# samiwilf/torchrec-oldfork

Hardware: AMD Instinct MI355X
Metric: samples/sec Criteo-1TB DLRM batch 65536 (higher is better)
Workload: dtype f32; 1 GPU; DLRM Criteo-1TB shape: 26 tables (177.9M rows, 84.85 GiB fp32, D=128), 13 dense, pooling factor 1, dense 512-256-128, over 1024-1024-512-256-1, fused exact SGD; global_batch=65536, local_batch=65536, parallelism=mp1: 26 table-wise + 0 row-wise + 0 replicated (data-parallel) tables, dense dp1, ids=uniform, distinct_batches=32, seed=0, data_ranks=1

## Files before the change

### torchrec-oldfork_amd/csrc/dlrm_interaction.hip

```cpp
#include <algorithm>
#include <cstdlib>

#include "common.hpp"

namespace tbe {

using f32x4 = __attribute__((ext_vector_type(4))) float;

__device__ __forceinline__ void wave_lds_fence() { __builtin_amdgcn_wave_barrier(); }

__device__ __forceinline__ int triu_index(int i, int j, int R) { return i * (2 * R - i - 1) / 2 + (j - i - 1); }

__device__ __forceinline__ int triu_row(int p, int R) {
  const int t = 2 * R - 1;
  int i = static_cast<int>((static_cast<float>(t) - sqrtf(static_cast<float>(t * t - 8 * p))) * 0.5f);
  i = max(0, min(i, R - 2));
  while (i + 1 <= R - 2 && (i + 1) * (2 * R - (i + 1) - 1) / 2 <= p) ++i;
  while (i > 0 && i * (2 * R - i - 1) / 2 > p) --i;
  return i;
}

template <int D>
struct XLoader {
  static constexpr int LOG_V = (D == 16 ? 2 : D == 32 ? 3 : D == 64 ? 4 : D == 128 ? 5 : 6);
  __device__ static __forceinline__ const float* src(const float* dense, const float* sparse, int64_t b, int F, int v) {
    const int r = v >> LOG_V;
    const int c = (v & ((1 << LOG_V) - 1)) * 4;
    return r == 0 ? dense + b * D + c : sparse + (b * F + (r - 1)) * D + c;
  }
};

template <int D>
__global__ __launch_bounds__(256, (D <= 128 ? 4 : 2)) void interaction_fwd_kernel(const float* __restrict__ dense,
                                                                                  const float* __restrict__ sparse,
                                                                                  float* __restrict__ out, int B, int F,
                                                                                  int64_t out_stride) {
  extern __shared__ float smem[];
  constexpr int NS = D / 16;
  const int lane = threadIdx.x & 63;
  const int wave = threadIdx.x >> 6;
  const int R = F + 1;
  const int P = R * (R - 1) / 2;
  const int P4 = (P + 3) & ~3;
  float* zs = smem + wave * P4;
  const bool vec_out = (out_stride & 3) == 0 && out_stride >= D + P4 && (reinterpret_cast<uintptr_t>(out) & 15) == 0;
  if (lane < P4 - P) zs[P + lane] = 0.f;
  const int r16 = lane & 15;
  const int kq = lane >> 4;
  const int row0 = min(r16, R - 1);
  const int row1 = min(16 + r16, R - 1);
  const int stride_b = gridDim.x * 4;
  float4 xa[NS], xb[NS];
  float4 dpass = make_float4(0.f, 0.f, 0.f, 0.f);
  auto issue_loads = [&](int b) {
    const float* x0 = (row0 == 0 ? dense + static_cast<int64_t>(b) * D
                                 : sparse + (static_cast<int64_t>(b) * F + (row0 - 1)) * D) + 4 * kq;
    const float* x1 = sparse + (static_cast<int64_t>(b) * F + (row1 - 1)) * D + 4 * kq;
#pragma unroll
    for (int s = 0; s < NS; ++s) xa[s] = ld4(x0 + 16 * s);
    if (R > 16) {
#pragma unroll
      for (int s = 0; s < NS; ++s) xb[s] = ld4(x1 + 16 * s);
    } else {
#pragma unroll
      for (int s = 0; s < NS; ++s) xb[s] = make_float4(0.f, 0.f, 0.f, 0.f);
    }
    if (lane < D / 4) dpass = ld4(dense + static_cast<int64_t>(b) * D + lane * 4);
  };
  int b = blockIdx.x * 4 + wave;
  if (b < B) issue_loads(b);
  for (; b < B; b += stride_b) {
    f32x4 acc00 = {0.f, 0.f, 0.f, 0.f}, acc01 = acc00, acc11 = acc00;
#pragma unroll
    for (int s = 0; s < NS; ++s) {
      const float a0[4] = {xa[s].x, xa[s].y, xa[s].z, xa[s].w};
      const float a1[4] = {xb[s].x, xb[s].y, xb[s].z, xb[s].w};
#pragma unroll
      for (int e = 0; e < 4; ++e) {
        acc00 = __builtin_amdgcn_mfma_f32_16x16x4f32(a0[e], a0[e], acc00, 0, 0, 0);
        acc01 = __builtin_amdgcn_mfma_f32_16x16x4f32(a0[e], a1[e], acc01, 0, 0, 0);
        acc11 = __builtin_amdgcn_mfma_f32_16x16x4f32(a1[e], a1[e], acc11, 0, 0, 0);
      }
    }
    float* orow = out + static_cast<int64_t>(b) * out_stride;
    if (lane < D / 4) {
      if (vec_out) {
        st4(orow + lane * 4, dpass);
      } else {
        orow[lane * 4 + 0] = dpass.x;
        orow[lane * 4 + 1] = dpass.y;
        orow[lane * 4 + 2] = dpass.z;
        orow[lane * 4 + 3] = dpass.w;
      }
    }
    if (b + stride_b < B) issue_loads(b + stride_b);
#pragma unroll
    for (int q = 0; q < 4; ++q) {
      const int i = kq * 4 + q;
      const int j = r16;
      if (i < j && j < R) zs[triu_index(i, j, R)] = acc00[q];
      if (16 + j < R && i < R) zs[triu_index(i, 16 + j, R)] = acc01[q];
      if (i < j && 16 + j < R) zs[triu_index(16 + i, 16 + j, R)] = acc11[q];
    }
    __builtin_amdgcn_wave_barrier();
    constexpr int MAXT = 8;
    constexpr int MAXQ = 2;
    if (vec_out) {
#pragma unroll
      for (int t = 0; t < MAXQ; ++t) {
        const int q = lane + t * kWave;
        if (q < P4 / 4) st4(orow + D + 4 * q, *reinterpret_cast<const float4*>(zs + 4 * q));
      }
    } else {
#pragma unroll
      for (int t = 0; t < MAXT; ++t) {
        const int p = lane + t * kWave;
        if (p < P) orow[D + p] = zs[p];
      }
    }
    __builtin_amdgcn_wave_barrier();
  }
}

__device__ __forceinline__ void vm_store_dword(float* p, float v) {
  asm volatile("global_store_dword %0, %1, off" ::"v"(p), "v"(v) : "memory");
}

template <int N>
__device__ __forceinline__ void vm_wait_all_but() {
  asm volatile("s_waitcnt vmcnt(%0)" ::"n"(N) : "memory");
}

__device__ __forceinline__ void vm_wait_all_but(int n) {
  switch (n) {
    case 1: vm_wait_all_but<1>(); break;
    case 2: vm_wait_all_but<2>(); break;
    case 3: vm_wait_all_but<3>(); break;
    case 4: vm_wait_all_but<4>(); break;
    case 5: vm_wait_all_but<5>(); break;
    case 6: vm_wait_all_but<6>(); break;
    case 7: vm_wait_all_but<7>(); break;
    case 8: vm_wait_all_but<8>(); break;
    case 9: vm_wait_all_but<9>(); break;
    case 10: vm_wait_all_but<10>(); break;
    case 11: vm_wait_all_but<11>(); break;
    case 12: vm_wait_all_but<12>(); break;
    default: vm_wait_all_but<0>(); break;
  }
}

template <int D>
__global__ __launch_bounds__(256, 2) void interaction_fwd_glds_kernel(const float* __restrict__ dense,
                                                                     const float* __restrict__ sparse,
                                                                     float* __restrict__ out, int B, int F,
                                                                     int64_t out_stride) {
  extern __shared__ float smem[];
  constexpr int NS = D / 16;
  constexpr int PR = D / 4;
  constexpr int RPI = kWave / PR;
  constexpr int MAXI = 32 / RPI;
  static_assert(PR >= 16 && PR <= kWave, "LDS-DMA form needs 64 <= D <= 256");
  const int lane = threadIdx.x & 63;
  const int wave = threadIdx.x >> 6;
  const int R = F + 1;
  const int P = R * (R - 1) / 2;
  const int P4 = (P + 3) & ~3;
  const int NI = (R + RPI - 1) / RPI;
  float* xs = smem + wave * (NI * RPI * D + P4);
  float* zs = xs + NI * RPI * D;
  const bool vec_out = (out_stride & 3) == 0 && out_stride >= D + P4 && (reinterpret_cast<uintptr_t>(out) & 15) == 0;
  if (lane < P4 - P) zs[P + lane] = 0.f;
  const int r16 = lane & 15;
  const int kq = lane >> 4;
  const int row0 = min(r16, R - 1);
  const int row1 = min(16 + r16, R - 1);
  const int stride_b = gridDim.x * 4;
  int src_off[MAXI];
#pragma unroll
  for (int i = 0; i < MAXI; ++i) {
    const int row = min(i * RPI + lane / PR, R - 1);
    const int piece = (lane % PR) ^ (row & 15);
    src_off[i] = (row - 1) * D + 4 * piece;
  }
  const bool dense_lane = lane < PR;
  auto issue_copy = [&](int b) {
    const float* sp = sparse + static_cast<int64_t>(b) * F * D;
    const float* dn = dense + static_cast<int64_t>(b) * D + D;
#pragma unroll
    for (int i = 0; i < MAXI; ++i) {
      if (i < NI) {
        const float* g = (i == 0 && dense_lane) ? dn + src_off[0] : sp + src_off[i];
        __builtin_amdgcn_global_load_lds((const __attribute__((address_space(1))) void*)g,
                                         (__attribute__((address_space(3))) void*)(xs + i * (kWave * 4)), 16, 0, 0);
      }
    }
  };
  const int T = (P + kWave - 1) / kWave;
  constexpr int DS = (D + kWave - 1) / kWave;
  int stores_behind_copy = 0;
  int b = blockIdx.x * 4 + wave;
  if (b < B) issue_copy(b);
  for (; b < B; b += stride_b) {
    vm_wait_all_but(stores_behind_copy);
    __builtin_amdgcn_wave_barrier();
    float4 xa[NS], xb[NS];
#pragma unroll
    for (int s = 0; s < NS; ++s) xa[s] = *reinterpret_cast<const float4*>(xs + row0 * D + 4 * ((4 * s + kq) ^ (row0 & 15)));
    if (R > 16) {
#pragma unroll
      for (int s = 0; s < NS; ++s) xb[s] = *reinterpret_cast<const float4*>(xs + row1 * D + 4 * ((4 * s + kq) ^ (row1 & 15)));
    } else {
#pragma unroll
      for (int s = 0; s < NS; ++s) xb[s] = make_float4(0.f, 0.f, 0.f, 0.f);
    }
    float4 dpass = make_float4(0.f, 0.f, 0.f, 0.f);
    float dscal[DS];
    if (vec_out) {
      if (dense_lane) dpass = *reinterpret_cast<const float4*>(xs + 4 * lane);
    } else {
#pragma unroll
      for (int t = 0; t < DS; ++t) dscal[t] = xs[min(lane + t * kWave, D - 1)];
    }
    asm volatile("s_waitcnt lgkmcnt(0)" ::: "memory");
    __builtin_amdgcn_wave_barrier();
    if (b + stride_b < B) issue_copy(b + stride_b);
    f32x4 acc00 = {0.f, 0.f, 0.f, 0.f}, acc01 = acc00, acc11 = acc00;
#pragma unroll
    for (int s = 0; s < NS; ++s) {
      const float a0[4] = {xa[s].x, xa[s].y, xa[s].z, xa[s].w};
      const float a1[4] = {xb[s].x, xb[s].y, xb[s].z, xb[s].w};
#pragma unroll
      for (int e = 0; e < 4; ++e) {
        acc00 = __builtin_amdgcn_mfma_f32_16x16x4f32(a0[e], a0[e], acc00, 0, 0, 0);
        acc01 = __builtin_amdgcn_mfma_f32_16x16x4f32(a0[e], a1[e], acc01, 0, 0, 0);
        acc11 = __builtin_amdgcn_mfma_f32_16x16x4f32(a1[e], a1[e], acc11, 0, 0, 0);
      }
    }
    float* orow = out + static_cast<int64_t>(b) * out_stride;
    if (vec_out) {
      if (dense_lane) st4(orow + lane * 4, dpass);
    } else {
#pragma unroll
      for (int t = 0; t < DS; ++t) vm_store_dword(orow + min(lane + t * kWave, D - 1), dscal[t]);
    }
#pragma unroll
    for (int q = 0; q < 4; ++q) {
      const int i = kq * 4 + q;
      const int j = r16;
      if (i < j && j < R) zs[triu_index(i, j, R)] = acc00[q];
      if (16 + j < R && i < R) zs[triu_index(i, 16 + j, R)] = acc01[q];
      if (i < j && 16 + j < R) zs[triu_index(16 + i, 16 + j, R)] = acc11[q];
    }
    __builtin_amdgcn_wave_barrier();
    constexpr int MAXT = 8;
    constexpr int MAXQ = 2;
    if (vec_out) {
#pragma unroll
      for (int t = 0; t < MAXQ; ++t) {
        const int q = lane + t * kWave;
        if (q < P4 / 4) st4(orow + D + 4 * q, *reinterpret_cast<const float4*>(zs + 4 * q));
      }
      stores_behind_copy = 0;
    } else {
      float zv[MAXT];
#pragma unroll
      for (int t = 0; t < MAXT; ++t)
        if (t < T) zv[t] = zs[min(lane + t * kWave, P - 1)];
#pragma unroll
      for (int t = 0; t < MAXT; ++t)
        if (t < T) vm_store_dword(orow + D + min(lane + t * kWave, P - 1), zv[t]);
      stores_behind_copy = DS + T;
    }
    __builtin_amdgcn_wave_barrier();
  }
}

template <int NT>
__global__ __launch_bounds__(256, 2) void interaction_bwd_kernel(const float* __restrict__ dense,
                                                                 const float* __restrict__ sparse,
                                                                 const float* __restrict__ grad_out,
                                                                 float* __restrict__ grad_dense,
                                                                 float* __restrict__ grad_sparse, int B, int F,
                                                                 int64_t grad_stride) {
  extern __shared__ float smem[];
  constexpr int D = NT * 16;
  constexpr int XS = D + 16;
  constexpr int GS = 34;
  constexpr int XROWS = 28;
  constexpr int LOG_V = XLoader<D>::LOG_V;
  constexpr int MAXV = (XROWS * D / 4 + kWave - 1) / kWave;
  const int lane = threadIdx.x & 63;
  const int wave = threadIdx.x >> 6;
  const int R = F + 1;
  const int P = R * (R - 1) / 2;
  float* xs = smem + wave * (XROWS * XS + 32 * GS);
  float* gs = xs + XROWS * XS;
  const int r16 = lane & 15;
  const int kq = lane >> 4;
  const int nvec = R * (D / 4);
  const int ksteps = (R + 3) / 4;
  const int stride_b = gridDim.x * 4;
  for (int e = lane; e < XROWS * XS; e += kWave) xs[e] = 0.f;
  for (int e = lane; e < 32 * GS; e += kWave) gs[e] = 0.f;
  constexpr int MAXP = (28 * 27 / 2 + kWave - 1) / kWave;
  int pij[MAXP];
#pragma unroll
  for (int t = 0; t < MAXP; ++t) {
    const int p = lane + t * kWave;
    int i = 0, j = 1;
    if (p < P) {
      i = triu_row(p, R);
      j = i + 1 + (p - i * (2 * R - i - 1) / 2);
    }
    pij[t] = (i << 8) | j;
  }
  wave_lds_fence();

  float4 pre[MAXV];
  float gpre[MAXP];
  int b = blockIdx.x * 4 + wave;
  if (b < B) {
#pragma unroll
    for (int i = 0; i < MAXV; ++i) {
      const int v = lane + i * kWave;
      if (v < nvec) pre[i] = ld4(XLoader<D>::src(dense, sparse, b, F, v));
    }
#pragma unroll
    for (int t = 0; t < MAXP; ++t) {
      const int p = lane + t * kWave;
      gpre[t] = p < P ? grad_out[static_cast<int64_t>(b) * grad_stride + D + p] : 0.f;
    }
  }
  for (; b < B; b += stride_b) {
#pragma unroll
    for (int i = 0; i < MAXV; ++i) {
      const int v = lane + i * kWave;
      if (v < nvec) st4(xs + (v >> LOG_V) * XS + (v & ((1 << LOG_V) - 1)) * 4, pre[i]);
    }
#pragma unroll
    for (int t = 0; t < MAXP; ++t) {
      if (lane + t * kWave < P) {
        const int i = pij[t] >> 8, j = pij[t] & 255;
        gs[i * GS + j] = gpre[t];
        gs[j * GS + i] = gpre[t];
      }
    }
    const float* grow = grad_out + static_cast<int64_t>(b) * grad_stride;
    float4 gdense = make_float4(0.f, 0.f, 0.f, 0.f);
    if (lane < D / 4) {
      if (((grad_stride & 3) | (reinterpret_cast<uintptr_t>(grad_out) & 15)) == 0) {
        gdense = ld4(grow + lane * 4);
      } else {
        gdense.x = grow[lane * 4 + 0];
        gdense.y = grow[lane * 4 + 1];
        gdense.z = grow[lane * 4 + 2];
        gdense.w = grow[lane * 4 + 3];
      }
    }
    const int nb = b + stride_b;
    if (nb < B) {
#pragma unroll
      for (int i = 0; i < MAXV; ++i) {
        const int v = lane + i * kWave;
        if (v < nvec) pre[i] = ld4(XLoader<D>::src(dense, sparse, nb, F, v));
      }
#pragma unroll
      for (int t = 0; t < MAXP; ++t) {
        const int p = lane + t * kWave;
        gpre[t] = p < P ? grad_out[static_cast<int64_t>(nb) * grad_stride + D + p] : 0.f;
      }
    }
    wave_lds_fence();
    f32x4 acc[2][NT];
#pragma unroll
    for (int m = 0; m < 2; ++m)
#pragma unroll
      for (int n = 0; n < NT; ++n) acc[m][n] = f32x4{0.f, 0.f, 0.f, 0.f};
    for (int ks = 0; ks < ksteps; ++ks) {
      const int k = ks * 4 + kq;
      const float a0 = gs[r16 * GS + k];
      const float a1 = gs[(16 + r16) * GS + k];
      const float* xrow = xs + k * XS + r16;
#pragma unroll
      for (int n = 0; n < NT; ++n) {
        const float bn = xrow[16 * n];
        acc[0][n] = __builtin_amdgcn_mfma_f32_16x16x4f32(a0, bn, acc[0][n], 0, 0, 0);
        acc[1][n] = __builtin_amdgcn_mfma_f32_16x16x4f32(a1, bn, acc[1][n], 0, 0, 0);
      }
    }
    wave_lds_fence();
#pragma unroll
    for (int m = 0; m < 2; ++m)
#pragma unroll
      for (int n = 0; n < NT; ++n)
#pragma unroll
        for (int q = 0; q < 4; ++q) {
          const int row = 16 * m + 4 * kq + q;
          if (row < R) xs[row * XS + 16 * n + r16] = acc[m][n][q];
        }
    wave_lds_fence();
#pragma unroll
    for (int i = 0; i < MAXV; ++i) {
      const int v = lane + i * kWave;
      if (v < nvec) {
        const int r = v >> LOG_V;
        const int c = (v & ((1 << LOG_V) - 1)) * 4;
        float4 x = ld4(xs + r * XS + c);
        if (r == 0) {
          x.x += gdense.x;
          x.y += gdense.y;
          x.z += gdense.z;
          x.w += gdense.w;
          st4(grad_dense + static_cast<int64_t>(b) * D + c, x);
        } else {
          st4(grad_sparse + (static_cast<int64_t>(b) * F + (r - 1)) * D + c, x);
        }
      }
    }
    wave_lds_fence();
  }
}


__device__ __attribute__((aligned(16))) float g_zero_row[256];

struct GatherLane {
  RowWindow win;
  uint64_t base;
  bool counts;
};
__device__ __forceinline__ GatherLane load_gather_lane(const uint64_t* feat_weights, const int64_t* feat_rows,
                                                       const int64_t* feat_window, int lane, int F) {
  GatherLane g;
  const int f = min(lane, F - 1);
  g.win = load_window(feat_rows, feat_window, f);
  g.base = feat_weights[f];
  g.counts = lane < F;
  return g;
}
template <int D>
__device__ __forceinline__ uint64_t gather_row_address(const GatherLane& g, int64_t id, uint64_t miss, int& nbad) {
  int64_t local;
  const int cls = classify_id(g.win, id, local);
  if (cls == kIdBad && g.counts) ++nbad;
  return cls == kIdLocal ? g.base + static_cast<uint64_t>(local) * (D * sizeof(float)) : miss;
}
__device__ __forceinline__ void report_bad_ids(int nbad, int32_t* bounds_errors) {
  if (bounds_errors == nullptr) return;
#pragma unroll
  for (int o = 32; o > 0; o >>= 1) nbad += __shfl_xor(nbad, o, kWave);
  if ((threadIdx.x & 63) == 0 && nbad > 0) atomicAdd(bounds_errors, nbad);
}

template <int D>
__global__ __launch_bounds__(256, 2) void interaction_gather_fwd_kernel(const float* __restrict__ dense,
                                                                       const uint64_t* __restrict__ feat_weights,
                                                                       const int64_t* __restrict__ feat_rows,
                                                                       const int64_t* __restrict__ feat_window,
                                                                       const int64_t* __restrict__ indices,
                                                                       float* __restrict__ out,
                                                                       int32_t* __restrict__ bounds_errors, int B, int F,
                                                                       int64_t out_stride) {
  extern __shared__ float smem[];
  constexpr int NS = D / 16;
  constexpr int PR = D / 4;
  constexpr int RPI = kWave / PR;
  constexpr int IDS = 64;
  static_assert(PR >= 16 && PR <= kWave, "LDS-DMA form needs 64 <= D <= 256");
  const int lane = threadIdx.x & 63;
  const int wave = threadIdx.x >> 6;
  const int R = F + 1;
  const int P = R * (R - 1) / 2;
  const int P4 = (P + 3) & ~3;
  const int NI = (R + RPI - 1) / RPI;
  float* xs = smem + wave * (NI * RPI * D + P4 + IDS);
  float* zs = xs + NI * RPI * D;
  float* ids = zs + P4;
  const bool vec_out = (out_stride & 3) == 0 && out_stride >= D + P4 && (reinterpret_cast<uintptr_t>(out) & 15) == 0;
  if (lane < P4 - P) zs[P + lane] = 0.f;
  const int r16 = lane & 15;
  const int kq = lane >> 4;
  const int row0 = min(r16, R - 1);
  const int row1 = min(16 + r16, R - 1);
  const int stride_b = gridDim.x * 4;
  const GatherLane gl = load_gather_lane(feat_weights, feat_rows, feat_window, lane, F);
  const uint64_t zero_row = reinterpret_cast<uint64_t>(&g_zero_row[0]);
  int nbad = 0;
  const uint32_t* id_words = reinterpret_cast<const uint32_t*>(indices) +
                             2 * static_cast<int64_t>(min(lane >> 1, F - 1)) * B + (lane & 1);
  auto issue_ids = [&](int b) {
    __builtin_amdgcn_global_load_lds((const __attribute__((address_space(1))) void*)(id_words + 2 * static_cast<int64_t>(b)),
                                     (__attribute__((address_space(3))) void*)ids, 4, 0, 0);
  };
  auto issue_copy = [&](int b, uint64_t row_addr) {
    const uint64_t dn = reinterpret_cast<uint64_t>(dense + static_cast<int64_t>(b) * D);
#pragma unroll 1
    for (int i = 0; i < NI; ++i) {
      const int row = min(i * RPI + lane / PR, R - 1);
      const int piece = (lane % PR) ^ (row & 15);
      uint64_t src = shflu64(row_addr, max(row - 1, 0));
      if (row == 0) src = dn;
      src += 16 * piece;
      __builtin_amdgcn_global_load_lds((const __attribute__((address_space(1))) void*)src,
                                       (__attribute__((address_space(3))) void*)(xs + i * (kWave * 4)), 16, 0, 0);
    }
  };
  auto read_id = [&]() { return *reinterpret_cast<const int64_t*>(ids + 2 * min(lane, F - 1)); };
  const bool dense_lane = lane < PR;
  const int T = (P + kWave - 1) / kWave;
  constexpr int DS = (D + kWave - 1) / kWave;
  int stores_behind_copy = 0;
  int b = blockIdx.x * 4 + wave;
  if (b < B) {
    issue_ids(b);
    vm_wait_all_but<0>();
    __builtin_amdgcn_wave_barrier();
    const int64_t id = read_id();
    asm volatile("s_waitcnt lgkmcnt(0)" ::: "memory");
    __builtin_amdgcn_wave_barrier();
    issue_copy(b, gather_row_address<D>(gl, id, zero_row, nbad));
    if (b + stride_b < B) issue_ids(b + stride_b);
  }
  for (; b < B; b += stride_b) {
    vm_wait_all_but(stores_behind_copy);
    __builtin_amdgcn_wave_barrier();
    float4 xa[NS], xb[NS];
#pragma unroll
    for (int s = 0; s < NS; ++s) xa[s] = *reinterpret_cast<const float4*>(xs + row0 * D + 4 * ((4 * s + kq) ^ (row0 & 15)));
    if (R > 16) {
#pragma unroll
      for (int s = 0; s < NS; ++s) xb[s] = *reinterpret_cast<const float4*>(xs + row1 * D + 4 * ((4 * s + kq) ^ (row1 & 15)));
    } else {
#pragma unroll
      for (int s = 0; s < NS; ++s) xb[s] = make_float4(0.f, 0.f, 0.f, 0.f);
    }
    float4 dpass = make_float4(0.f, 0.f, 0.f, 0.f);
    float dscal[DS];
    if (vec_out) {
      if (dense_lane) dpass = *reinterpret_cast<const float4*>(xs + 4 * lane);
    } else {
#pragma unroll
      for (int t = 0; t < DS; ++t) dscal[t] = xs[min(lane + t * kWave, D - 1)];
    }
    const int64_t next_id = read_id();
    asm volatile("s_waitcnt lgkmcnt(0)" ::: "memory");
    __builtin_amdgcn_wave_barrier();
    if (b + stride_b < B) {
      issue_copy(b + stride_b, gather_row_address<D>(gl, next_id, zero_row, nbad));
      if (b + 2 * stride_b < B) issue_ids(b + 2 * stride_b);
    }
    f32x4 acc00 = {0.f, 0.f, 0.f, 0.f}, acc01 = acc00, acc11 = acc00;
#pragma unroll
    for (int s = 0; s < NS; ++s) {
      const float a0[4] = {xa[s].x, xa[s].y, xa[s].z, xa[s].w};
      const float a1[4] = {xb[s].x, xb[s].y, xb[s].z, xb[s].w};
#pragma unroll
      for (int e = 0; e < 4; ++e) {
        acc00 = __builtin_amdgcn_mfma_f32_16x16x4f32(a0[e], a0[e], acc00, 0, 0, 0);
        acc01 = __builtin_amdgcn_mfma_f32_16x16x4f32(a0[e], a1[e], acc01, 0, 0, 0);
        acc11 = __builtin_amdgcn_mfma_f32_16x16x4f32(a1[e], a1[e], acc11, 0, 0, 0);
      }
    }
    float* orow = out + static_cast<int64_t>(b) * out_stride;
    if (vec_out) {
      if (dense_lane) st4(orow + lane * 4, dpass);
    } else {
#pragma unroll
      for (int t = 0; t < DS; ++t) vm_store_dword(orow + min(lane + t * kWave, D - 1), dscal[t]);
    }
#pragma unroll
    for (int q = 0; q < 4; ++q) {
      const int i = kq * 4 + q;
      const int j = r16;
      if (i < j && j < R) zs[triu_index(i, j, R)] = acc00[q];
      if (16 + j < R && i < R) zs[triu_index(i, 16 + j, R)] = acc01[q];
      if (i < j && 16 + j < R) zs[triu_index(16 + i, 16 + j, R)] = acc11[q];
    }
    __builtin_amdgcn_wave_barrier();
    constexpr int MAXT = 8;
    constexpr int MAXQ = 2;
    if (vec_out) {
#pragma unroll
      for (int t = 0; t < MAXQ; ++t) {
        const int q = lane + t * kWave;
        if (q < P4 / 4) st4(orow + D + 4 * q, *reinterpret_cast<const float4*>(zs + 4 * q));
      }
      stores_behind_copy = 0;
    } else {
      float zv[MAXT];
#pragma unroll
      for (int t = 0; t < MAXT; ++t)
        if (t < T) zv[t] = zs[min(lane + t * kWave, P - 1)];
#pragma unroll
      for (int t = 0; t < MAXT; ++t)
        if (t < T) vm_store_dword(orow + D + min(lane + t * kWave, P - 1), zv[t]);
      stores_behind_copy = DS + T;
    }
    __builtin_amdgcn_wave_barrier();
  }
  report_bad_ids(nbad, bounds_errors);
}

template <int NT, bool SGD = false>
__global__ __launch_bounds__(256, 2) void interaction_gather_bwd_kernel(const float* __restrict__ dense,
                                                                       const uint64_t* __restrict__ feat_weights,
                                                                       const int64_t* __restrict__ feat_rows,
                                                                       const int64_t* __restrict__ feat_window,
                                                                       const int64_t* __restrict__ indices,
                                                                       const float* __restrict__ grad_out,
                                                                       float* __restrict__ grad_dense,
                                                                       float* __restrict__ grad_sparse,
                                                                       int32_t* __restrict__ bounds_errors, int B, int F,
                                                                       int64_t grad_stride,
                                                                       const uint8_t* __restrict__ single, float lr) {
  extern __shared__ float smem[];
  constexpr int D = NT * 16;
  constexpr int XS = D + 16;
  constexpr int GS = 34;
  constexpr int XROWS = 28;
  constexpr int LOG_V = XLoader<D>::LOG_V;
  constexpr int MAXV = (XROWS * D / 4 + kWave - 1) / kWave;
  const int lane = threadIdx.x & 63;
  const int wave = threadIdx.x >> 6;
  const int R = F + 1;
  const int P = R * (R - 1) / 2;
  float* xs = smem + wave * (XROWS * XS + 32 * GS);
  float* gs = xs + XROWS * XS;
  const int r16 = lane & 15;
  const int kq = lane >> 4;
  const int nvec = R * (D / 4);
  const int ksteps = (R + 3) / 4;
  const int stride_b = gridDim.x * 4;
  for (int e = lane; e < XROWS * XS; e += kWave) xs[e] = 0.f;
  for (int e = lane; e < 32 * GS; e += kWave) gs[e] = 0.f;
  constexpr int MAXP = (28 * 27 / 2 + kWave - 1) / kWave;
  int pij[MAXP];
#pragma unroll
  for (int t = 0; t < MAXP; ++t) {
    const int p = lane + t * kWave;
    int i = 0, j = 1;
    if (p < P) {
      i = triu_row(p, R);
      j = i + 1 + (p - i * (2 * R - i - 1) / 2);
    }
    pij[t] = (i << 8) | j;
  }
  wave_lds_fence();

  const GatherLane gl = load_gather_lane(feat_weights, feat_rows, feat_window, lane, F);
  const int64_t* my_ids = indices + static_cast<int64_t>(min(lane, F - 1)) * B;
  auto my_single = [&](int s) { return single[(my_ids + s) - indices]; };
  uint32_t once_in_flight = 0;
  uint32_t next_single = 0;
  int slot = 0;
  auto publish_once = [&](uint64_t row_addr, uint32_t flag, int into_slot) {
    const bool once = lane < F && row_addr != 0 && flag != 0;
    if (lane < F) reinterpret_cast<uint64_t*>(xs + (lane + 1) * XS + D)[into_slot] = once ? row_addr : 0;
    return static_cast<uint32_t>(__ballot(once));
  };
  int nbad = 0;
  float4 pre[MAXV];
  float gpre[MAXP];
  auto load_x = [&](int s, uint64_t row_addr) {
#pragma unroll
    for (int i = 0; i < MAXV; ++i) {
      const int v = lane + i * kWave;
      const int r = min(v >> LOG_V, R - 1);
      const int c = (v & ((1 << LOG_V) - 1)) * 4;
      const uint64_t src = shflu64(row_addr, max(r - 1, 0));
      if (v < nvec) {
        if (r == 0)
          pre[i] = ld4(dense + static_cast<int64_t>(s) * D + c);
        else
          pre[i] = src != 0 ? ld4(reinterpret_cast<const float*>(src) + c) : make_float4(0.f, 0.f, 0.f, 0.f);
      }
    }
  };
  int b = blockIdx.x * 4 + wave;
  int64_t next_id = 0;
  if (b < B) {
    const uint64_t row_addr = gather_row_address<D>(gl, my_ids[b], 0, nbad);
    if constexpr (SGD) once_in_flight = publish_once(row_addr, my_single(b), 0);
    load_x(b, row_addr);
    if (b + stride_b < B) {
      next_id = my_ids[b + stride_b];
      if constexpr (SGD) next_single = my_single(b + stride_b);
    }
#pragma unroll
    for (int t = 0; t < MAXP; ++t) {
      const int p = lane + t * kWave;
      gpre[t] = p < P ? grad_out[static_cast<int64_t>(b) * grad_stride + D + p] : 0.f;
    }
  }
  for (; b < B; b += stride_b) {
    const uint32_t once_b = once_in_flight << 1;
#pragma unroll
    for (int i = 0; i < MAXV; ++i) {
      const int v = lane + i * kWave;
      if (v < nvec) st4(xs + (v >> LOG_V) * XS + (v & ((1 << LOG_V) - 1)) * 4, pre[i]);
    }
#pragma unroll
    for (int t = 0; t < MAXP; ++t) {
      if (lane + t * kWave < P) {
        const int i = pij[t] >> 8, j = pij[t] & 255;
        gs[i * GS + j] = gpre[t];
        gs[j * GS + i] = gpre[t];
      }
    }
    const float* grow = grad_out + static_cast<int64_t>(b) * grad_stride;
    float4 gdense = make_float4(0.f, 0.f, 0.f, 0.f);
    if (lane < D / 4) {
      if (((grad_stride & 3) | (reinterpret_cast<uintptr_t>(grad_out) & 15)) == 0) {
        gdense = ld4(grow + lane * 4);
      } else {
        gdense.x = grow[lane * 4 + 0];
        gdense.y = grow[lane * 4 + 1];
        gdense.z = grow[lane * 4 + 2];
        gdense.w = grow[lane * 4 + 3];
      }
    }
    const int nb = b + stride_b;
    if (nb < B) {
      const uint64_t row_addr = gather_row_address<D>(gl, next_id, 0, nbad);
      if constexpr (SGD) once_in_flight = publish_once(row_addr, next_single, slot ^ 1);
      load_x(nb, row_addr);
      if (nb + stride_b < B) {
        next_id = my_ids[nb + stride_b];
        if constexpr (SGD) next_single = my_single(nb + stride_b);
      }
#pragma unroll
      for (int t = 0; t < MAXP; ++t) {
        const int p = lane + t * kWave;
        gpre[t] = p < P ? grad_out[static_cast<int64_t>(nb) * grad_stride + D + p] : 0.f;
      }
    }
    wave_lds_fence();
    f32x4 acc[2][NT];
#pragma unroll
    for (int m = 0; m < 2; ++m)
#pragma unroll
      for (int n = 0; n < NT; ++n) acc[m][n] = f32x4{0.f, 0.f, 0.f, 0.f};
    for (int ks = 0; ks < ksteps; ++ks) {
      const int k = ks * 4 + kq;
      const float a0 = gs[r16 * GS + k];
      const float a1 = gs[(16 + r16) * GS + k];
      const float* xrow = xs + k * XS + r16;
#pragma unroll
      for (int n = 0; n < NT; ++n) {
        const float bn = xrow[16 * n];
        acc[0][n] = __builtin_amdgcn_mfma_f32_16x16x4f32(a0, bn, acc[0][n], 0, 0, 0);
        acc[1][n] = __builtin_amdgcn_mfma_f32_16x16x4f32(a1, bn, acc[1][n], 0, 0, 0);
      }
    }
    wave_lds_fence();
    if constexpr (SGD) {
#pragma unroll
      for (int m = 0; m < 2; ++m)
#pragma unroll
        for (int q = 0; q < 4; ++q) {
          const int row = 16 * m + 4 * kq + q;
          if (row < R) {
            float* xw = xs + row * XS + r16;
            const bool once = ((once_b >> row) & 1u) != 0;
            float w[NT];
#pragma unroll
            for (int n = 0; n < NT; ++n) w[n] = xw[16 * n];
#pragma unroll
            for (int n = 0; n < NT; ++n) {
              const float g = acc[m][n][q];
              xw[16 * n] = once ? fmaf(-lr, fmaf(1.f, g, 0.f), w[n]) : g;
            }
          }
        }
    } else {
#pragma unroll
      for (int m = 0; m < 2; ++m)
#pragma unroll
        for (int n = 0; n < NT; ++n)
#pragma unroll
          for (int q = 0; q < 4; ++q) {
            const int row = 16 * m + 4 * kq + q;
            if (row < R) xs[row * XS + 16 * n + r16] = acc[m][n][q];
          }
    }
    wave_lds_fence();
    if constexpr (SGD) {
      constexpr int RPV = kWave >> LOG_V;
      const int r0 = lane >> LOG_V;
      const int c0 = (lane & ((1 << LOG_V) - 1)) * 4;
      const float* xl = xs + r0 * XS + c0;
      const uint64_t* sl = reinterpret_cast<const uint64_t*>(xs + r0 * XS + D) + slot;
      float* gsl = grad_sparse + (static_cast<int64_t>(b) * F - 1) * D + 4 * lane;
#pragma unroll
      for (int i = 0; i < MAXV; ++i) {
        const int r = r0 + i * RPV;
        if (r < R) {
          float4 x = ld4(xl + i * RPV * XS);
          if (i == 0 && r == 0) {
            x.x += gdense.x;
            x.y += gdense.y;
            x.z += gdense.z;
            x.w += gdense.w;
            st4(grad_dense + static_cast<int64_t>(b) * D + c0, x);
          } else {
            const uint64_t table_row = sl[i * RPV * (XS / 2)];
            st4(table_row != 0 ? reinterpret_cast<float*>(table_row) + c0 : gsl + i * (4 * kWave), x);
          }
        }
      }
    } else {
#pragma unroll
      for (int i = 0; i < MAXV; ++i) {
        const int v = lane + i * kWave;
        if (v < nvec) {
          const int r = v >> LOG_V;
          const int c = (v & ((1 << LOG_V) - 1)) * 4;
          float4 x = ld4(xs + r * XS + c);
          if (r == 0) {
            x.x += gdense.x;
            x.y += gdense.y;
            x.z += gdense.z;
            x.w += gdense.w;
            st4(grad_dense + static_cast<int64_t>(b) * D + c, x);
          } else {
            st4(grad_sparse + (static_cast<int64_t>(b) * F + (r - 1)) * D + c, x);
          }
        }
      }
    }
    wave_lds_fence();
    slot ^= 1;
  }
  report_bad_ids(nbad, bounds_errors);
}

}

using namespace tbe;

static unsigned interaction_grid(int B) {
  const int64_t want = (static_cast<int64_t>(B) + 3) / 4;
  return static_cast<unsigned>(std::max<int64_t>(1, std::min<int64_t>(want, 256 * 2)));
}

template <typename K>
static bool reserve_lds(K kernel, size_t bytes) {
  return hipFuncSetAttribute(reinterpret_cast<const void*>(kernel), hipFuncAttributeMaxDynamicSharedMemorySize,
                             static_cast<int>(bytes)) == hipSuccess;
}

extern "C" int tbe_dlrm_interaction_forward_f32(const float* dense, const float* sparse, int32_t B, int32_t F,
                                                int32_t D, float* out, int64_t out_row_stride, void* stream) {
  TBE_REQUIRE(B >= 0 && F >= 1 && F <= 31, "tbe_dlrm_interaction_forward_f32: F=%d outside [1, 31]", F);
  TBE_REQUIRE(out_row_stride >= D + (F + 1) * F / 2, "tbe_dlrm_interaction_forward_f32: out_row_stride %lld < D + F(F+1)/2",
              (long long)out_row_stride);
  TBE_REQUIRE(D == 16 || D == 32 || D == 64 || D == 128 || D == 256,
              "tbe_dlrm_interaction_forward_f32: D=%d not in {16,32,64,128,256}", D);
  if (B == 0) return TBE_OK;
  TBE_REQUIRE(dense && sparse && out, "tbe_dlrm_interaction_forward_f32: null pointer");
  TBE_REQUIRE(((reinterpret_cast<uintptr_t>(dense) | reinterpret_cast<uintptr_t>(sparse)) & 15) == 0,
              "tbe_dlrm_interaction_forward_f32: inputs must be 16-B aligned");
  const int R = F + 1, P = R * (R - 1) / 2;
  const size_t lds = 4 * static_cast<size_t>((P + 3) & ~3) * sizeof(float);
  hipStream_t st = static_cast<hipStream_t>(stream);
  const int64_t want = (static_cast<int64_t>(B) + 3) / 4;
  const dim3 grid(static_cast<unsigned>(std::max<int64_t>(1, std::min<int64_t>(want, 256 * (D <= 128 ? 4 : 2)))));
  if (D == 64 || D == 128) {
    const int rpi = 64 / (D / 4);
    const int rows = (R + rpi - 1) / rpi * rpi;
    const size_t lds_g = 4 * (static_cast<size_t>(rows) * D + ((P + 3) & ~3)) * sizeof(float);
    static bool glds_attr = false;
    if (!glds_attr) {
      const size_t big = 4 * (static_cast<size_t>(32) * 128 + 496) * sizeof(float);
      if (!reserve_lds(interaction_fwd_glds_kernel<128>, big) || !reserve_lds(interaction_fwd_glds_kernel<64>, big)) {
        set_error("tbe_dlrm_interaction_forward_f32: cannot reserve LDS");
        return TBE_ERR_LAUNCH;
      }
      glds_attr = true;
    }
    const dim3 grid_g(static_cast<unsigned>(std::max<int64_t>(1, std::min<int64_t>(want, 256 * 2))));
    if (D == 128)
      hipLaunchKernelGGL(interaction_fwd_glds_kernel<128>, grid_g, dim3(256), lds_g, st, dense, sparse, out, B, F, out_row_stride);
    else
      hipLaunchKernelGGL(interaction_fwd_glds_kernel<64>, grid_g, dim3(256), lds_g, st, dense, sparse, out, B, F, out_row_stride);
    TBE_CHECK_LAUNCH("tbe_dlrm_interaction_forward_f32");
    return TBE_OK;
  }
#define TBE_IF(DD) hipLaunchKernelGGL(interaction_fwd_kernel<DD>, grid, dim3(256), lds, st, dense, sparse, out, B, F, out_row_stride)
  switch (D) {
    case 16: TBE_IF(16); break;
    case 32: TBE_IF(32); break;
    default: TBE_IF(256); break;
  }
#undef TBE_IF
  TBE_CHECK_LAUNCH("tbe_dlrm_interaction_forward_f32");
  return TBE_OK;
}

extern "C" int tbe_dlrm_interaction_backward_f32(const float* dense, const float* sparse, const float* grad_out,
                                                 int64_t grad_row_stride, int32_t B, int32_t F, int32_t D,
                                                 float* grad_dense, float* grad_sparse, void* stream) {
  TBE_REQUIRE(B >= 0 && F >= 1 && F <= 27, "tbe_dlrm_interaction_backward_f32: F=%d outside [1, 27]", F);
  TBE_REQUIRE(grad_row_stride >= D + (F + 1) * F / 2, "tbe_dlrm_interaction_backward_f32: grad_row_stride %lld < D + F(F+1)/2",
              (long long)grad_row_stride);
  TBE_REQUIRE(D == 16 || D == 32 || D == 64 || D == 128, "tbe_dlrm_interaction_backward_f32: D=%d not in {16,32,64,128}", D);
  if (B == 0) return TBE_OK;
  TBE_REQUIRE(dense && sparse && grad_out && grad_dense && grad_sparse, "tbe_dlrm_interaction_backward_f32: null pointer");
  TBE_REQUIRE(((reinterpret_cast<uintptr_t>(dense) | reinterpret_cast<uintptr_t>(sparse) |
                reinterpret_cast<uintptr_t>(grad_dense) | reinterpret_cast<uintptr_t>(grad_sparse)) & 15) == 0,
              "tbe_dlrm_interaction_backward_f32: tensors must be 16-B aligned");
  hipStream_t st = static_cast<hipStream_t>(stream);
  const size_t lds = 4 * (static_cast<size_t>(28) * (D + 16) + 32 * 34) * sizeof(float);
  const dim3 grid(interaction_grid(B));
  static bool attr_set = false;
  if (!attr_set) {
    const size_t big = 4 * (28 * (128 + 16) + 32 * 34) * sizeof(float);
    if (!reserve_lds(interaction_bwd_kernel<8>, big) || !reserve_lds(interaction_bwd_kernel<4>, big)) {
      set_error("tbe_dlrm_interaction_backward_f32: cannot reserve LDS");
      return TBE_ERR_LAUNCH;
    }
    attr_set = true;
  }
#define TBE_IB(NT) \
  hipLaunchKernelGGL(interaction_bwd_kernel<NT>, grid, dim3(256), lds, st, dense, sparse, grad_out, grad_dense, grad_sparse, B, F, grad_row_stride)
  switch (D) {
    case 16: TBE_IB(1); break;
    case 32: TBE_IB(2); break;
    case 64: TBE_IB(4); break;
    default: TBE_IB(8); break;
  }
#undef TBE_IB
  TBE_CHECK_LAUNCH("tbe_dlrm_interaction_backward_f32");
  return TBE_OK;
}

static int check_gather_args(const char* what, int32_t B, int32_t F, int32_t D, int64_t row_stride) {
  TBE_REQUIRE(B >= 0 && F >= 1 && F <= 27, "%s: F=%d outside [1, 27]", what, F);
  TBE_REQUIRE(D == 64 || D == 128, "%s: D=%d not in {64,128}", what, D);
  TBE_REQUIRE(row_stride >= D + (F + 1) * F / 2, "%s: row stride %lld < D + F(F+1)/2", what, (long long)row_stride);
  return TBE_OK;
}

extern "C" int tbe_dlrm_interaction_gather_forward_f32(const float* dense, const uint64_t* feat_weights,
                                                       const int64_t* feat_rows, const int64_t* feat_window,
                                                       const int64_t* indices, int32_t B, int32_t F, int32_t D, float* out,
                                                       int64_t out_row_stride, int32_t* bounds_errors, void* stream) {
  const char* what = "tbe_dlrm_interaction_gather_forward_f32";
  if (int rc = check_gather_args(what, B, F, D, out_row_stride)) return rc;
  TBE_REQUIRE(dense && feat_weights && feat_rows && indices && out, "%s: null pointer", what);
  TBE_REQUIRE((reinterpret_cast<uintptr_t>(dense) & 15) == 0 && (reinterpret_cast<uintptr_t>(indices) & 7) == 0,
              "%s: dense must be 16-B aligned, indices 8-B aligned", what);
  if (B == 0) return TBE_OK;
  const int R = F + 1, P = R * (R - 1) / 2;
  const int rpi = 64 / (D / 4);
  const int rows = (R + rpi - 1) / rpi * rpi;
  const size_t lds = 4 * (static_cast<size_t>(rows) * D + ((P + 3) & ~3) + 64) * sizeof(float);
  static bool attr_set = false;
  if (!attr_set) {
    const size_t big = 4 * (static_cast<size_t>(28) * 128 + 380 + 64) * sizeof(float);
    if (!reserve_lds(interaction_gather_fwd_kernel<128>, big) || !reserve_lds(interaction_gather_fwd_kernel<64>, big)) {
      set_error("%s: cannot reserve LDS", what);
      return TBE_ERR_LAUNCH;
    }
    attr_set = true;
  }
  hipStream_t st = static_cast<hipStream_t>(stream);
  const dim3 grid(interaction_grid(B));
  if (D == 128)
    hipLaunchKernelGGL(interaction_gather_fwd_kernel<128>, grid, dim3(256), lds, st, dense, feat_weights, feat_rows,
                       feat_window, indices, out, bounds_errors, B, F, out_row_stride);
  else
    hipLaunchKernelGGL(interaction_gather_fwd_kernel<64>, grid, dim3(256), lds, st, dense, feat_weights, feat_rows,
                       feat_window, indices, out, bounds_errors, B, F, out_row_stride);
  TBE_CHECK_LAUNCH(what);
  return TBE_OK;
}

extern "C" int tbe_dlrm_interaction_gather_backward_f32(const float* dense, const uint64_t* feat_weights,
                                                        const int64_t* feat_rows, const int64_t* feat_window,
                                                        const int64_t* indices, const float* grad_out,
                                                        int64_t grad_row_stride, int32_t B, int32_t F, int32_t D,
                                                        float* grad_dense, float* grad_sparse, int32_t* bounds_errors,
                                                        void* stream) {
  const char* what = "tbe_dlrm_interaction_gather_backward_f32";
  if (int rc = check_gather_args(what, B, F, D, grad_row_stride)) return rc;
  TBE_REQUIRE(dense && feat_weights && feat_rows && indices && grad_out && grad_dense && grad_sparse, "%s: null pointer",
              what);
  TBE_REQUIRE(((reinterpret_cast<uintptr_t>(dense) | reinterpret_cast<uintptr_t>(grad_dense) |
                reinterpret_cast<uintptr_t>(grad_sparse)) & 15) == 0 && (reinterpret_cast<uintptr_t>(indices) & 7) == 0,
              "%s: tensors must be 16-B aligned, indices 8-B aligned", what);
  if (B == 0) return TBE_OK;
  hipStream_t st = static_cast<hipStream_t>(stream);
  const size_t lds = 4 * (static_cast<size_t>(28) * (D + 16) + 32 * 34) * sizeof(float);
  static bool attr_set = false;
  if (!attr_set) {
    const size_t big = 4 * (28 * (128 + 16) + 32 * 34) * sizeof(float);
    if (!reserve_lds(interaction_gather_bwd_kernel<8>, big) || !reserve_lds(interaction_gather_bwd_kernel<4>, big)) {
      set_error("%s: cannot reserve LDS", what);
      return TBE_ERR_LAUNCH;
    }
    attr_set = true;
  }
  const dim3 grid(interaction_grid(B));
  const uint8_t* const no_flags = nullptr;
  if (D == 128)
    hipLaunchKernelGGL(interaction_gather_bwd_kernel<8>, grid, dim3(256), lds, st, dense, feat_weights, feat_rows,
                       feat_window, indices, grad_out, grad_dense, grad_sparse, bounds_errors, B, F, grad_row_stride,
                       no_flags, 0.f);
  else
    hipLaunchKernelGGL(interaction_gather_bwd_kernel<4>, grid, dim3(256), lds, st, dense, feat_weights, feat_rows,
                       feat_window, indices, grad_out, grad_dense, grad_sparse, bounds_errors, B, F, grad_row_stride,
                       no_flags, 0.f);
  TBE_CHECK_LAUNCH(what);
  return TBE_OK;
}

extern "C" int tbe_dlrm_interaction_gather_backward_sgd_f32(const float* dense, const uint64_t* feat_weights,
                                                            const int64_t* feat_rows, const int64_t* feat_window,
                                                            const int64_t* indices, const float* grad_out,
                                                            int64_t grad_row_stride, int32_t B, int32_t F, int32_t D,
                                                            float* grad_dense, float* grad_sparse,
                                                            int32_t* bounds_errors, const uint8_t* single,
                                                            float learning_rate, void* stream) {
  const char* what = "tbe_dlrm_interaction_gather_backward_sgd_f32";
  if (int rc = check_gather_args(what, B, F, D, grad_row_stride)) return rc;
  TBE_REQUIRE(dense && feat_weights && feat_rows && indices && grad_out && grad_dense && grad_sparse && single,
              "%s: null pointer", what);
  TBE_REQUIRE(((reinterpret_cast<uintptr_t>(dense) | reinterpret_cast<uintptr_t>(grad_dense) |
                reinterpret_cast<uintptr_t>(grad_sparse)) & 15) == 0 && (reinterpret_cast<uintptr_t>(indices) & 7) == 0,
              "%s: tensors must be 16-B aligned, indices 8-B aligned", what);
  if (B == 0) return TBE_OK;
  hipStream_t st = static_cast<hipStream_t>(stream);
  const size_t lds = 4 * (static_cast<size_t>(28) * (D + 16) + 32 * 34) * sizeof(float);
  static bool attr_set = false;
  if (!attr_set) {
    const size_t big = 4 * (28 * (128 + 16) + 32 * 34) * sizeof(float);
    if (!reserve_lds(interaction_gather_bwd_kernel<8, true>, big) || !reserve_lds(interaction_gather_bwd_kernel<4, true>, big)) {
      set_error("%s: cannot reserve LDS", what);
      return TBE_ERR_LAUNCH;
    }
    attr_set = true;
  }
  const dim3 grid(interaction_grid(B));
  if (D == 128)
    hipLaunchKernelGGL((interaction_gather_bwd_kernel<8, true>), grid, dim3(256), lds, st, dense, feat_weights, feat_rows,
                       feat_window, indices, grad_out, grad_dense, grad_sparse, bounds_errors, B, F, grad_row_stride,
                       single, learning_rate);
  else
    hipLaunchKernelGGL((interaction_gather_bwd_kernel<4, true>), grid, dim3(256), lds, st, dense, feat_weights, feat_rows,
                       feat_window, indices, grad_out, grad_dense, grad_sparse, bounds_errors, B, F, grad_row_stride,
                       single, learning_rate);
  TBE_CHECK_LAUNCH(what);
  return TBE_OK;
}
```

Before: 8.214 million samples/s.

## Defer interaction forward output stores by one iteration behind next copy issue

```diff
diff --git a/torchrec-oldfork_amd/csrc/dlrm_interaction.hip b/torchrec-oldfork_amd/csrc/dlrm_interaction.hip
--- a/torchrec-oldfork_amd/csrc/dlrm_interaction.hip
+++ b/torchrec-oldfork_amd/csrc/dlrm_interaction.hip
@@ -122,30 +122,49 @@
   }
 }
 
-__device__ __forceinline__ void vm_store_dword(float* p, float v) {
-  asm volatile("global_store_dword %0, %1, off" ::"v"(p), "v"(v) : "memory");
-}
-
-template <int N>
-__device__ __forceinline__ void vm_wait_all_but() {
-  asm volatile("s_waitcnt vmcnt(%0)" ::"n"(N) : "memory");
-}
-
-__device__ __forceinline__ void vm_wait_all_but(int n) {
-  switch (n) {
-    case 1: vm_wait_all_but<1>(); break;
-    case 2: vm_wait_all_but<2>(); break;
-    case 3: vm_wait_all_but<3>(); break;
-    case 4: vm_wait_all_but<4>(); break;
-    case 5: vm_wait_all_but<5>(); break;
-    case 6: vm_wait_all_but<6>(); break;
-    case 7: vm_wait_all_but<7>(); break;
-    case 8: vm_wait_all_but<8>(); break;
-    case 9: vm_wait_all_but<9>(); break;
-    case 10: vm_wait_all_but<10>(); break;
-    case 11: vm_wait_all_but<11>(); break;
-    case 12: vm_wait_all_but<12>(); break;
-    default: vm_wait_all_but<0>(); break;
+__device__ __forceinline__ void vm_wait_all() { asm volatile("s_waitcnt vmcnt(0)" ::: "memory"); }
+__device__ __forceinline__ void lds_wait_all() { asm volatile("s_waitcnt lgkmcnt(0)" ::: "memory"); }
+
+struct PendingRow {
+  float* row;
+  float dd[4];
+  float zv[8];
+};
+
+__device__ __forceinline__ void pending_read_pairs(PendingRow& p, const float* zs, bool vec_out, int lane, int P, int P4) {
+  if (vec_out) {
+#pragma unroll
+    for (int t = 0; t < 2; ++t) {
+      const int q = lane + t * kWave;
+      if (q < P4 / 4) {
+        const float4 v = *reinterpret_cast<const float4*>(zs + 4 * q);
+        p.zv[4 * t + 0] = v.x, p.zv[4 * t + 1] = v.y, p.zv[4 * t + 2] = v.z, p.zv[4 * t + 3] = v.w;
+      }
+    }
+  } else {
+    const int T = (P + kWave - 1) / kWave;
+#pragma unroll
+    for (int t = 0; t < 8; ++t)
+      if (t < T) p.zv[t] = zs[min(lane + t * kWave, P - 1)];
+  }
+}
+
+template <int D>
+__device__ __forceinline__ void pending_store(const PendingRow& p, bool vec_out, int lane, int P, int P4) {
+  if (vec_out) {
+    if (lane < D / 4) st4(p.row + 4 * lane, make_float4(p.dd[0], p.dd[1], p.dd[2], p.dd[3]));
+#pragma unroll
+    for (int t = 0; t < 2; ++t) {
+      const int q = lane + t * kWave;
+      if (q < P4 / 4) st4(p.row + D + 4 * q, make_float4(p.zv[4 * t], p.zv[4 * t + 1], p.zv[4 * t + 2], p.zv[4 * t + 3]));
+    }
+  } else {
+    const int T = (P + kWave - 1) / kWave;
+#pragma unroll
+    for (int t = 0; t < D / kWave; ++t) p.row[lane + t * kWave] = p.dd[t];
+#pragma unroll
+    for (int t = 0; t < 8; ++t)
+      if (t < T) p.row[D + min(lane + t * kWave, P - 1)] = p.zv[t];
   }
 }
 
@@ -195,13 +214,13 @@
       }
     }
   };
-  const int T = (P + kWave - 1) / kWave;
-  constexpr int DS = (D + kWave - 1) / kWave;
-  int stores_behind_copy = 0;
-  int b = blockIdx.x * 4 + wave;
+  constexpr int DS = D / kWave;
+  const int first_b = blockIdx.x * 4 + wave;
+  int b = first_b;
   if (b < B) issue_copy(b);
+  PendingRow pend;
   for (; b < B; b += stride_b) {
-    vm_wait_all_but(stores_behind_copy);
+    vm_wait_all();
     __builtin_amdgcn_wave_barrier();
     float4 xa[NS], xb[NS];
 #pragma unroll
@@ -213,16 +232,19 @@
 #pragma unroll
       for (int s = 0; s < NS; ++s) xb[s] = make_float4(0.f, 0.f, 0.f, 0.f);
     }
-    float4 dpass = make_float4(0.f, 0.f, 0.f, 0.f);
-    float dscal[DS];
+    float dd[4] = {0.f, 0.f, 0.f, 0.f};
     if (vec_out) {
-      if (dense_lane) dpass = *reinterpret_cast<const float4*>(xs + 4 * lane);
+      if (dense_lane) {
+        const float4 v = *reinterpret_cast<const float4*>(xs + 4 * lane);
+        dd[0] = v.x, dd[1] = v.y, dd[2] = v.z, dd[3] = v.w;
+      }
     } else {
 #pragma unroll
-      for (int t = 0; t < DS; ++t) dscal[t] = xs[min(lane + t * kWave, D - 1)];
-    }
-    asm volatile("s_waitcnt lgkmcnt(0)" ::: "memory");
-    __builtin_amdgcn_wave_barrier();
+      for (int t = 0; t < DS; ++t) dd[t] = xs[lane + t * kWave];
+    }
+    lds_wait_all();
+    __builtin_amdgcn_wave_barrier();
+    if (b != first_b) pending_store<D>(pend, vec_out, lane, P, P4);
     if (b + stride_b < B) issue_copy(b + stride_b);
     f32x4 acc00 = {0.f, 0.f, 0.f, 0.f}, acc01 = acc00, acc11 = acc00;
 #pragma unroll
@@ -235,13 +257,6 @@
         acc01 = __builtin_amdgcn_mfma_f32_16x16x4f32(a0[e], a1[e], acc01, 0, 0, 0);
         acc11 = __builtin_amdgcn_mfma_f32_16x16x4f32(a1[e], a1[e], acc11, 0, 0, 0);
       }
-    }
-    float* orow = out + static_cast<int64_t>(b) * out_stride;
-    if (vec_out) {
-      if (dense_lane) st4(orow + lane * 4, dpass);
-    } else {
-#pragma unroll
-      for (int t = 0; t < DS; ++t) vm_store_dword(orow + min(lane + t * kWave, D - 1), dscal[t]);
     }
 #pragma unroll
     for (int q = 0; q < 4; ++q) {
@@ -252,27 +267,13 @@
       if (i < j && 16 + j < R) zs[triu_index(16 + i, 16 + j, R)] = acc11[q];
     }
     __builtin_amdgcn_wave_barrier();
-    constexpr int MAXT = 8;
-    constexpr int MAXQ = 2;
-    if (vec_out) {
-#pragma unroll
-      for (int t = 0; t < MAXQ; ++t) {
-        const int q = lane + t * kWave;
-        if (q < P4 / 4) st4(orow + D + 4 * q, *reinterpret_cast<const float4*>(zs + 4 * q));
-      }
-      stores_behind_copy = 0;
-    } else {
-      float zv[MAXT];
-#pragma unroll
-      for (int t = 0; t < MAXT; ++t)
-        if (t < T) zv[t] = zs[min(lane + t * kWave, P - 1)];
-#pragma unroll
-      for (int t = 0; t < MAXT; ++t)
-        if (t < T) vm_store_dword(orow + D + min(lane + t * kWave, P - 1), zv[t]);
-      stores_behind_copy = DS + T;
-    }
-    __builtin_amdgcn_wave_barrier();
-  }
+    pend.row = out + static_cast<int64_t>(b) * out_stride;
+#pragma unroll
+    for (int t = 0; t < 4; ++t) pend.dd[t] = dd[t];
+    pending_read_pairs(pend, zs, vec_out, lane, P, P4);
+    __builtin_amdgcn_wave_barrier();
+  }
+  if (first_b < B) pending_store<D>(pend, vec_out, lane, P, P4);
 }
 
 template <int NT>
@@ -507,22 +508,22 @@
   };
   auto read_id = [&]() { return *reinterpret_cast<const int64_t*>(ids + 2 * min(lane, F - 1)); };
   const bool dense_lane = lane < PR;
-  const int T = (P + kWave - 1) / kWave;
-  constexpr int DS = (D + kWave - 1) / kWave;
-  int stores_behind_copy = 0;
-  int b = blockIdx.x * 4 + wave;
+  constexpr int DS = D / kWave;
+  const int first_b = blockIdx.x * 4 + wave;
+  int b = first_b;
   if (b < B) {
     issue_ids(b);
-    vm_wait_all_but<0>();
+    vm_wait_all();
     __builtin_amdgcn_wave_barrier();
     const int64_t id = read_id();
-    asm volatile("s_waitcnt lgkmcnt(0)" ::: "memory");
+    lds_wait_all();
     __builtin_amdgcn_wave_barrier();
     issue_copy(b, gather_row_address<D>(gl, id, zero_row, nbad));
     if (b + stride_b < B) issue_ids(b + stride_b);
   }
+  PendingRow pend;
   for (; b < B; b += stride_b) {
-    vm_wait_all_but(stores_behind_copy);
+    vm_wait_all();
     __builtin_amdgcn_wave_barrier();
     float4 xa[NS], xb[NS];
 #pragma unroll
@@ -534,17 +535,20 @@
 #pragma unroll
       for (int s = 0; s < NS; ++s) xb[s] = make_float4(0.f, 0.f, 0.f, 0.f);
     }
-    float4 dpass = make_float4(0.f, 0.f, 0.f, 0.f);
-    float dscal[DS];
+    float dd[4] = {0.f, 0.f, 0.f, 0.f};
     if (vec_out) {
-      if (dense_lane) dpass = *reinterpret_cast<const float4*>(xs + 4 * lane);
+      if (dense_lane) {
+        const float4 v = *reinterpret_cast<const float4*>(xs + 4 * lane);
+        dd[0] = v.x, dd[1] = v.y, dd[2] = v.z, dd[3] = v.w;
+      }
     } else {
 #pragma unroll
-      for (int t = 0; t < DS; ++t) dscal[t] = xs[min(lane + t * kWave, D - 1)];
+      for (int t = 0; t < DS; ++t) dd[t] = xs[lane + t * kWave];
     }
     const int64_t next_id = read_id();
-    asm volatile("s_waitcnt lgkmcnt(0)" ::: "memory");
-    __builtin_amdgcn_wave_barrier();
+    lds_wait_all();
+    __builtin_amdgcn_wave_barrier();
+    if (b != first_b) pending_store<D>(pend, vec_out, lane, P, P4);
     if (b + stride_b < B) {
       issue_copy(b + stride_b, gather_row_address<D>(gl, next_id, zero_row, nbad));
       if (b + 2 * stride_b < B) issue_ids(b + 2 * stride_b);
@@ -560,13 +564,6 @@
         acc01 = __builtin_amdgcn_mfma_f32_16x16x4f32(a0[e], a1[e], acc01, 0, 0, 0);
         acc11 = __builtin_amdgcn_mfma_f32_16x16x4f32(a1[e], a1[e], acc11, 0, 0, 0);
       }
-    }
-    float* orow = out + static_cast<int64_t>(b) * out_stride;
-    if (vec_out) {
-      if (dense_lane) st4(orow + lane * 4, dpass);
-    } else {
-#pragma unroll
-      for (int t = 0; t < DS; ++t) vm_store_dword(orow + min(lane + t * kWave, D - 1), dscal[t]);
     }
 #pragma unroll
     for (int q = 0; q < 4; ++q) {
@@ -577,27 +574,13 @@
       if (i < j && 16 + j < R) zs[triu_index(16 + i, 16 + j, R)] = acc11[q];
     }
     __builtin_amdgcn_wave_barrier();
-    constexpr int MAXT = 8;
-    constexpr int MAXQ = 2;
-    if (vec_out) {
-#pragma unroll
-      for (int t = 0; t < MAXQ; ++t) {
-        const int q = lane + t * kWave;
-        if (q < P4 / 4) st4(orow + D + 4 * q, *reinterpret_cast<const float4*>(zs + 4 * q));
-      }
-      stores_behind_copy = 0;
-    } else {
-      float zv[MAXT];
-#pragma unroll
-      for (int t = 0; t < MAXT; ++t)
-        if (t < T) zv[t] = zs[min(lane + t * kWave, P - 1)];
-#pragma unroll
-      for (int t = 0; t < MAXT; ++t)
-        if (t < T) vm_store_dword(orow + D + min(lane + t * kWave, P - 1), zv[t]);
-      stores_behind_copy = DS + T;
-    }
-    __builtin_amdgcn_wave_barrier();
-  }
+    pend.row = out + static_cast<int64_t>(b) * out_stride;
+#pragma unroll
+    for (int t = 0; t < 4; ++t) pend.dd[t] = dd[t];
+    pending_read_pairs(pend, zs, vec_out, lane, P, P4);
+    __builtin_amdgcn_wave_barrier();
+  }
+  if (first_b < B) pending_store<D>(pend, vec_out, lane, P, P4);
   report_bad_ids(nbad, bounds_errors);
 }
 
```

Measured after the change: 8.197 million samples/s. Within noise of the previous version (-0.2%).
